# bdina9/qat-vit

Hardware: AMD Instinct MI355X
Metric: images/sec QAT student step (fwd+bwd+allreduce) (higher is better)
Workload: dtype f32 (emulated: int8 MFMA for grid x grid products; forward float operands as fp16 hi+lo pairs; backward gradients as ONE fp16 plane scaled per tensor - 2^-12 per element, <= 4e-4 relative L2 per stage against the fp32 reference, bf16-pair fallback on overflow; fp32 / exact-integer accumulate)

## Files before the change

qat-vit_amd/csrc/f16strip.hip:

```cpp
#include <stdlib.h>

#include "qv_common.h"
#include "qv_kernels.h"

namespace qv {

typedef int i32x4 __attribute__((ext_vector_type(4)));
typedef float f32x4 __attribute__((ext_vector_type(4)));
typedef _Float16 f16x8 __attribute__((ext_vector_type(8)));
typedef __attribute__((address_space(3))) void lds_void;

struct F16StripArgs {
    const _Float16* A;
    const i32x4* Bf;
    int M, N, lda;
    const float* s1;
    const float* s2;
    const float* qp;
    int qmin, qmax;
    const float* colscale;
    const uint8_t* code8;
    const uint8_t* mask;
    int ldc;
    _Float16* out;
    const float* o16_mul;
    uint32_t* o16_amax;
};

typedef int v4i32 __attribute__((ext_vector_type(4)));
__device__ inline v4i32 fs_rsrc(const void* base, int64_t bytes) {
    const uint64_t b = reinterpret_cast<uint64_t>(base);
    const uint32_t n = bytes > 0xffffffffll ? 0xffffffffu : (uint32_t)bytes;
    return (v4i32){(int)(uint32_t)b, (int)(uint32_t)(b >> 32), (int)n, 0x00020000};
}
__device__ inline void fs_dma16(v4i32 rsrc, const char* lds_dst, uint32_t voff) {
    const uint32_t m = __builtin_amdgcn_readfirstlane((uint32_t)reinterpret_cast<uintptr_t>((lds_void*)lds_dst));
    uint32_t keep;
    asm volatile("s_mov_b32 %0, m0\n\ts_mov_b32 m0, %2\n\ts_nop 0\n\tbuffer_load_dwordx4 %1, %3, 0 offen lds\n\ts_mov_b32 m0, %0"
                 : "=&s"(keep)
                 : "v"(voff), "s"(m), "s"(rsrc)
                 : "memory");
}

__device__ inline int fstrip_off(int row, int chunk) {
    const int R = row >> 1;
    return R * 128 + (((((row & 1) << 2) | chunk) ^ (R & 7)) << 4);
}

template <int NTL>
__global__ __launch_bounds__(768, 3) void k_f16_strip_gelu_bwd(const F16StripArgs p) {
    constexpr int NWV = 12, TM = 7, TNT = 2, WC = 32, BMV = 104, KT = 12, PF = 3, NT_ = NWV * 64, BN = 384;
    constexpr int IMGA = 16 * TM * 64, LA = KT * IMGA;
    constexpr int NC = NTL * BN;
    constexpr int WCODE = 16 * TM * WC;
    constexpr int CH = 1, OROW = 80, WOUT = 16 * CH * OROW;
    extern __shared__ __attribute__((aligned(16))) char smem[];
    char* sA = smem;
    float* sCs = reinterpret_cast<float*>(smem + LA);
    float* sLut = sCs + NC;
    char* sCodeAll = reinterpret_cast<char*>(sLut + 256);
    char* sOutAll = sCodeAll + NWV * WCODE;
    const int tid = threadIdx.x, lane = tid & 63;
    const int wave = __builtin_amdgcn_readfirstlane(tid >> 6);
    const int r = lane & 15, g = lane >> 4;
    const int m0 = blockIdx.x * BMV;

    {
        const int64_t abytes = (int64_t)p.M * p.lda * 2;
        const __amdgpu_buffer_rsrc_t rA = __builtin_amdgcn_make_buffer_rsrc(const_cast<_Float16*>(p.A), 0, abytes > 0xffffffffll ? 0xffffffffu : (uint32_t)abytes, 0x00020000);
        const int lR = lane >> 3, lL = (lane & 7) ^ lR;
        const int prow = 2 * lR + (lL >> 2), pk = lL & 3;
#pragma unroll
        for (int kt = 0; kt < KT; ++kt) {
            const int q = wave;
            if (q < TM) {
                const uint32_t off = (uint32_t)(((int64_t)(m0 + q * 16 + prow) * p.lda) * 2 + kt * 64 + pk * 16);
                __builtin_amdgcn_raw_ptr_buffer_load_lds(rA, (lds_void*)(sA + kt * IMGA + q * 1024), 16, off, 0, 0, 0);
            }
        }
    }
    const __amdgpu_buffer_rsrc_t rB = __builtin_amdgcn_make_buffer_rsrc(const_cast<i32x4*>(p.Bf), 0, (uint32_t)((int64_t)p.N * (KT * 64)), 0x00020000);
    const int f0 = wave * TNT;
    auto load_b = [&](int nt, int kt, i32x4 (&b)[TNT]) {
#pragma unroll
        for (int j = 0; j < TNT; ++j) {
            const int f = f0 + nt * 24 + j;
            const auto v = __builtin_amdgcn_raw_buffer_load_b128(rB, lane * 16, (((f / 3) * KT + kt) * 3 + f % 3) * 1024, 0);
            b[j] = __builtin_bit_cast(i32x4, v);
        }
    };
    i32x4 bb[2][TNT];
    load_b(0, 0, bb[0]);
    const v4i32 rC = fs_rsrc(p.code8, (int64_t)p.M * p.ldc);
    char* const sCode = sCodeAll + wave * WCODE;
    auto load_codes = [&](int nt) {
#pragma unroll
        for (int pc = 0; pc < 4; ++pc) {
            const int row = pc * 32 + (lane >> 1);
            if (pc < 3 || lane < 32) {
                const uint32_t off = (uint32_t)((int64_t)(m0 + row) * p.ldc + nt * BN + wave * WC + (lane & 1) * 16);
                fs_dma16(rC, sCode + pc * 1024, off);
            }
        }
    };
    load_codes(0);
    for (int c = tid; c < NC; c += NT_) sCs[c] = p.colscale ? p.colscale[c] : 1.0f;
    if (tid <= p.qmax - p.qmin) sLut[tid] = gelu_bwd(((float)(tid + p.qmin) - p.qp[2]) * p.qp[0]);
    const float alpha = (p.s1 ? *p.s1 : 1.0f) * (p.s2 ? *p.s2 : 1.0f);
    const float mul = *p.o16_mul;
    float am = 0.f;
    asm volatile("s_waitcnt vmcnt(0) lgkmcnt(0)" ::: "memory");
    __builtin_amdgcn_s_barrier();
    asm volatile("" ::: "memory");

    f32x4 acc[TM][TNT];
#pragma clang loop unroll(disable)
    for (int nt = 0; nt < NTL; ++nt) {
        auto kstep = [&](int kt, const i32x4 (&bc)[TNT]) {
            __builtin_amdgcn_sched_barrier(0);
            int opaque = 0;
            asm volatile("" : "+v"(opaque));
            const char* st = sA + opaque + kt * IMGA + fstrip_off(r, g);
            i32x4 af[PF];
#pragma unroll
            for (int i = 0; i < PF - 1; ++i) af[i] = *reinterpret_cast<const i32x4*>(st + 1024 * i);
#pragma unroll
            for (int i = 0; i < TM; ++i) {
                __builtin_amdgcn_sched_barrier(0);
                if (i + PF - 1 < TM) af[(i + PF - 1) % PF] = *reinterpret_cast<const i32x4*>(st + 1024 * (i + PF - 1));
#pragma unroll
                for (int j = 0; j < TNT; ++j)
                    acc[i][j] = __builtin_amdgcn_mfma_f32_16x16x32_f16(__builtin_bit_cast(f16x8, bc[j]), __builtin_bit_cast(f16x8, af[i % PF]),
                                                                       kt == 0 ? f32x4{0.f, 0.f, 0.f, 0.f} : acc[i][j], 0, 0, 0);
            }
        };
        __builtin_amdgcn_s_setprio(2);
#pragma unroll
        for (int kt = 0; kt < KT; ++kt) {
            if (kt + 1 < KT) load_b(nt, kt + 1, bb[(kt + 1) & 1]);
            else if (nt + 1 < NTL) load_b(nt + 1, 0, bb[0]);
            kstep(kt, bb[kt & 1]);
        }
        __builtin_amdgcn_sched_barrier(0);
        if (((wave >> 2) + nt) % 3 == 0) __builtin_amdgcn_s_setprio(1); else __builtin_amdgcn_s_setprio(0);

        int tid2 = threadIdx.x;
        asm volatile("" : "+v"(tid2));
        const int lane2 = tid2 & 63, r2 = lane2 & 15, g2 = lane2 >> 4;
        char* const sOut = sOutAll + wave * WOUT;
        const int colbase = nt * BN + wave * WC;
        uint32_t mword[TM];
#pragma unroll
        for (int i = 0; i < TM; ++i) {
            const int row = m0 + 16 * i + r2;
            mword[i] = row < p.M ? *reinterpret_cast<const uint32_t*>(p.mask + ((int64_t)row * p.ldc + colbase) / 8) : 0u;
        }
        asm volatile("s_waitcnt vmcnt(0)" ::: "memory");
#pragma unroll
        for (int c0 = 0; c0 < TM; c0 += CH) {
            const int nf = TM - c0 < CH ? TM - c0 : CH;
#pragma unroll
            for (int ii = 0; ii < CH; ++ii) {
                if (ii >= nf) continue;
                const int i = c0 + ii, rl = 16 * ii + r2;
#pragma unroll
                for (int j = 0; j < TNT; ++j) {
                    const uint32_t cd = *reinterpret_cast<const uint32_t*>(sCode + (16 * i + r2) * WC + 16 * j + 4 * g2);
                    const float4 cs = *reinterpret_cast<const float4*>(sCs + colbase + 16 * j + 4 * g2);
                    const float sv[4] = {cs.x, cs.y, cs.z, cs.w};
                    const uint32_t mb = mword[i] >> (16 * j + 4 * g2);
                    float o[4];
#pragma unroll
                    for (int e = 0; e < 4; ++e) {
                        const float v = acc[i][j][e] * alpha + 0.0f;
                        const float dg = sLut[(cd >> (8 * e)) & 0xffu];
                        o[e] = ((mb >> e) & 1u) ? v * dg * sv[e] : 0.f;
                    }
                    am = fmaxf(fmaxf(am, fmaxf(fabsf(o[0]), fabsf(o[1]))), fmaxf(fabsf(o[2]), fabsf(o[3])));
                    *reinterpret_cast<uint2*>(sOut + rl * OROW + (16 * j + 4 * g2) * 2) = make_uint2(pk_f16(o[0] * mul, o[1] * mul), pk_f16(o[2] * mul, o[3] * mul));
                }
            }
            asm volatile("s_waitcnt lgkmcnt(0)" ::: "memory");
            {
                const int rl = lane2 >> 2, c = lane2 & 3;
                const int lrow = 16 * c0 + rl, row = m0 + lrow;
                const uint4 v = *reinterpret_cast<const uint4*>(sOut + rl * OROW + 16 * c);
                if (lrow < BMV && row < p.M) *reinterpret_cast<uint4*>(p.out + (int64_t)row * p.ldc + colbase + 8 * c) = v;
            }
            asm volatile("" ::: "memory");
        }
        if (nt + 1 < NTL) {
            asm volatile("s_waitcnt lgkmcnt(0)" ::: "memory");
            load_codes(nt + 1);
        }
    }
    am = wave_max(am);
    if (lane == 0) atomicMax(p.o16_amax + (blockIdx.x & (kDyAmaxSlots - 1)) * kDyAmaxStride, __builtin_bit_cast(uint32_t, am));
}

bool launch_f16_strip_gelu_bwd(const void* A16, const void* B16f, float* , int M, int N, int K, int lda, int ldc, const float* s1, const float* s2, hipStream_t st,
                               const NTPost* post) {
    if (!knobs().f16_strip || !A16 || !B16f || !post || post->mode != 9 || K != 384 || N != 4 * 384 || lda % 8 != 0 || ldc % 128 != 0 || !post->qp || !post->out_hi ||
        !post->code8 || !post->code_mask || !post->o16_mul || !post->o16_amax || post->qmax - post->qmin >= 256)
        return false;
    if ((int64_t)M * lda * 2 >= (1ll << 32) || (int64_t)M * ldc >= (1ll << 32)) return false;
    F16StripArgs a{};
    a.A = reinterpret_cast<const _Float16*>(A16); a.Bf = reinterpret_cast<const i32x4*>(B16f); a.M = M; a.N = N; a.lda = lda; a.s1 = s1; a.s2 = s2;
    a.qp = post->qp; a.qmin = post->qmin; a.qmax = post->qmax; a.colscale = post->colscale;
    a.code8 = reinterpret_cast<const uint8_t*>(post->code8); a.mask = reinterpret_cast<const uint8_t*>(post->code_mask); a.ldc = ldc;
    a.out = reinterpret_cast<_Float16*>(post->out_hi); a.o16_mul = post->o16_mul; a.o16_amax = post->o16_amax;
    constexpr int kLds = 12 * 16 * 7 * 64 + 4 * 384 * 4 + 1024 + 12 * (16 * 7 * 32) + 12 * (16 * 80);
    static_assert(kLds <= 160 * 1024, "LDS");
    static bool once = ((void)hipFuncSetAttribute(reinterpret_cast<const void*>(k_f16_strip_gelu_bwd<4>), hipFuncAttributeMaxDynamicSharedMemorySize, kLds), true);
    (void)once;
    k_f16_strip_gelu_bwd<4><<<cdiv(M, 104), 768, kLds, st>>>(a);
    return true;
}

}
```

Baseline: 15800.

## Make f16 strip GELU-bwd kernel persistent with balanced strips and prefetch

Replaces the fixed grid of 104-row strips with a persistent grid capped at the CU count. Each block walks several equal-sized strips, with row count computed from M so the load balances across rounds. The next strip's A tile, first B fragment and codes are loaded during the epilogue of the current strip, and code reads and LUT gathers in the epilogue are software-pipelined. This aims to cut launch tail imbalance and expose prefetch overlap, at the cost of an extra barrier and more complex synchronization around reuse of shared memory.

```diff
diff --git a/qat-vit_amd/csrc/f16strip.hip b/qat-vit_amd/csrc/f16strip.hip
--- a/qat-vit_amd/csrc/f16strip.hip
+++ b/qat-vit_amd/csrc/f16strip.hip
@@ -14,6 +14,7 @@
     const _Float16* A;
     const i32x4* Bf;
     int M, N, lda;
+    int rows, strips;
     const float* s1;
     const float* s2;
     const float* qp;
@@ -49,11 +50,11 @@
 
 template <int NTL>
 __global__ __launch_bounds__(768, 3) void k_f16_strip_gelu_bwd(const F16StripArgs p) {
-    constexpr int NWV = 12, TM = 7, TNT = 2, WC = 32, BMV = 104, KT = 12, PF = 3, NT_ = NWV * 64, BN = 384;
+    constexpr int NWV = 12, TM = 7, TNT = 2, WC = 32, KT = 12, PF = 3, NT_ = NWV * 64, BN = 384;
     constexpr int IMGA = 16 * TM * 64, LA = KT * IMGA;
     constexpr int NC = NTL * BN;
     constexpr int WCODE = 16 * TM * WC;
-    constexpr int CH = 1, OROW = 80, WOUT = 16 * CH * OROW;
+    constexpr int OROW = 80, WOUT = 16 * OROW;
     extern __shared__ __attribute__((aligned(16))) char smem[];
     char* sA = smem;
     float* sCs = reinterpret_cast<float*>(smem + LA);
@@ -63,22 +64,18 @@
     const int tid = threadIdx.x, lane = tid & 63;
     const int wave = __builtin_amdgcn_readfirstlane(tid >> 6);
     const int r = lane & 15, g = lane >> 4;
-    const int m0 = blockIdx.x * BMV;
-
-    {
-        const int64_t abytes = (int64_t)p.M * p.lda * 2;
-        const __amdgpu_buffer_rsrc_t rA = __builtin_amdgcn_make_buffer_rsrc(const_cast<_Float16*>(p.A), 0, abytes > 0xffffffffll ? 0xffffffffu : (uint32_t)abytes, 0x00020000);
+    const int rows = p.rows;
+
+    const v4i32 rA = fs_rsrc(p.A, (int64_t)p.M * p.lda * 2);
+    auto load_strip = [&](int m0) {
         const int lR = lane >> 3, lL = (lane & 7) ^ lR;
         const int prow = 2 * lR + (lL >> 2), pk = lL & 3;
-#pragma unroll
-        for (int kt = 0; kt < KT; ++kt) {
-            const int q = wave;
-            if (q < TM) {
-                const uint32_t off = (uint32_t)(((int64_t)(m0 + q * 16 + prow) * p.lda) * 2 + kt * 64 + pk * 16);
-                __builtin_amdgcn_raw_ptr_buffer_load_lds(rA, (lds_void*)(sA + kt * IMGA + q * 1024), 16, off, 0, 0, 0);
-            }
-        }
-    }
+        if (wave < TM) {
+            const uint32_t base = (uint32_t)(((int64_t)(m0 + wave * 16 + prow) * p.lda) * 2 + pk * 16);
+#pragma unroll
+            for (int kt = 0; kt < KT; ++kt) fs_dma16(rA, sA + kt * IMGA + wave * 1024, base + kt * 64);
+        }
+    };
     const __amdgpu_buffer_rsrc_t rB = __builtin_amdgcn_make_buffer_rsrc(const_cast<i32x4*>(p.Bf), 0, (uint32_t)((int64_t)p.N * (KT * 64)), 0x00020000);
     const int f0 = wave * TNT;
     auto load_b = [&](int nt, int kt, i32x4 (&b)[TNT]) {
@@ -89,11 +86,9 @@
             b[j] = __builtin_bit_cast(i32x4, v);
         }
     };
-    i32x4 bb[2][TNT];
-    load_b(0, 0, bb[0]);
     const v4i32 rC = fs_rsrc(p.code8, (int64_t)p.M * p.ldc);
     char* const sCode = sCodeAll + wave * WCODE;
-    auto load_codes = [&](int nt) {
+    auto load_codes = [&](int m0, int nt) {
 #pragma unroll
         for (int pc = 0; pc < 4; ++pc) {
             const int row = pc * 32 + (lane >> 1);
@@ -103,96 +98,135 @@
             }
         }
     };
-    load_codes(0);
+    int s = blockIdx.x, m0 = s * rows;
+    load_strip(m0);
+    i32x4 bb[2][TNT];
+    load_b(0, 0, bb[0]);
+    load_codes(m0, 0);
     for (int c = tid; c < NC; c += NT_) sCs[c] = p.colscale ? p.colscale[c] : 1.0f;
     if (tid <= p.qmax - p.qmin) sLut[tid] = gelu_bwd(((float)(tid + p.qmin) - p.qp[2]) * p.qp[0]);
     const float alpha = (p.s1 ? *p.s1 : 1.0f) * (p.s2 ? *p.s2 : 1.0f);
     const float mul = *p.o16_mul;
     float am = 0.f;
-    asm volatile("s_waitcnt vmcnt(0) lgkmcnt(0)" ::: "memory");
-    __builtin_amdgcn_s_barrier();
-    asm volatile("" ::: "memory");
-
-    f32x4 acc[TM][TNT];
+
 #pragma clang loop unroll(disable)
-    for (int nt = 0; nt < NTL; ++nt) {
-        auto kstep = [&](int kt, const i32x4 (&bc)[TNT]) {
+    for (;;) {
+        asm volatile("s_waitcnt vmcnt(0) lgkmcnt(0)" ::: "memory");
+        __builtin_amdgcn_s_barrier();
+        asm volatile("" ::: "memory");
+        const int sn = s + (int)gridDim.x;
+        const bool more = sn < p.strips && sn * rows < p.M;
+        const int m1 = sn * rows;
+
+        f32x4 acc[TM][TNT];
+#pragma clang loop unroll(disable)
+        for (int nt = 0; nt < NTL; ++nt) {
+            auto kstep = [&](int kt, const i32x4 (&bc)[TNT]) {
+                __builtin_amdgcn_sched_barrier(0);
+                int opaque = 0;
+                asm volatile("" : "+v"(opaque));
+                const char* st = sA + opaque + kt * IMGA + fstrip_off(r, g);
+                i32x4 af[PF];
+#pragma unroll
+                for (int i = 0; i < PF - 1; ++i) af[i] = *reinterpret_cast<const i32x4*>(st + 1024 * i);
+#pragma unroll
+                for (int i = 0; i < TM; ++i) {
+                    __builtin_amdgcn_sched_barrier(0);
+                    if (i + PF - 1 < TM) af[(i + PF - 1) % PF] = *reinterpret_cast<const i32x4*>(st + 1024 * (i + PF - 1));
+#pragma unroll
+                    for (int j = 0; j < TNT; ++j)
+                        acc[i][j] = __builtin_amdgcn_mfma_f32_16x16x32_f16(__builtin_bit_cast(f16x8, bc[j]), __builtin_bit_cast(f16x8, af[i % PF]),
+                                                                           kt == 0 ? f32x4{0.f, 0.f, 0.f, 0.f} : acc[i][j], 0, 0, 0);
+                }
+            };
+            __builtin_amdgcn_s_setprio(2);
+#pragma unroll
+            for (int kt = 0; kt < KT; ++kt) {
+                if (kt + 1 < KT) load_b(nt, kt + 1, bb[(kt + 1) & 1]);
+                else if (nt + 1 < NTL || more) load_b(nt + 1 < NTL ? nt + 1 : 0, 0, bb[0]);
+                kstep(kt, bb[kt & 1]);
+            }
             __builtin_amdgcn_sched_barrier(0);
-            int opaque = 0;
-            asm volatile("" : "+v"(opaque));
-            const char* st = sA + opaque + kt * IMGA + fstrip_off(r, g);
-            i32x4 af[PF];
-#pragma unroll
-            for (int i = 0; i < PF - 1; ++i) af[i] = *reinterpret_cast<const i32x4*>(st + 1024 * i);
+            if (((wave >> 2) + nt) % 3 == 0) __builtin_amdgcn_s_setprio(1); else __builtin_amdgcn_s_setprio(0);
+
+            int tid2 = threadIdx.x;
+            asm volatile("" : "+v"(tid2));
+            const int lane2 = tid2 & 63, r2 = lane2 & 15, g2 = lane2 >> 4;
+            char* const sOut = sOutAll + wave * WOUT;
+            const int colbase = nt * BN + wave * WC;
+            uint32_t mword[TM];
 #pragma unroll
             for (int i = 0; i < TM; ++i) {
-                __builtin_amdgcn_sched_barrier(0);
-                if (i + PF - 1 < TM) af[(i + PF - 1) % PF] = *reinterpret_cast<const i32x4*>(st + 1024 * (i + PF - 1));
+                const int row = m0 + 16 * i + r2;
+                mword[i] = row < p.M ? *reinterpret_cast<const uint32_t*>(p.mask + ((int64_t)row * p.ldc + colbase) / 8) : 0u;
+            }
+            asm volatile("s_waitcnt vmcnt(0)" ::: "memory");
+#pragma unroll
+            for (int i = 0; i < TM; ++i) asm volatile("" : "+v"(mword[i]));
+            if (nt + 1 == NTL && more) {
+                __builtin_amdgcn_s_barrier();
+                asm volatile("" ::: "memory");
+                load_strip(m1);
+            }
+            float sv[TNT][4];
+#pragma unroll
+            for (int j = 0; j < TNT; ++j) {
+                const float4 cs = *reinterpret_cast<const float4*>(sCs + colbase + 16 * j + 4 * g2);
+                sv[j][0] = cs.x; sv[j][1] = cs.y; sv[j][2] = cs.z; sv[j][3] = cs.w;
+            }
+            uint32_t cd[TNT];
+            float dg[TNT][4];
+            auto read_codes = [&](int i) {
+#pragma unroll
+                for (int j = 0; j < TNT; ++j) cd[j] = *reinterpret_cast<const uint32_t*>(sCode + (16 * i + r2) * WC + 16 * j + 4 * g2);
+            };
+            auto gather = [&]() {
 #pragma unroll
                 for (int j = 0; j < TNT; ++j)
-                    acc[i][j] = __builtin_amdgcn_mfma_f32_16x16x32_f16(__builtin_bit_cast(f16x8, bc[j]), __builtin_bit_cast(f16x8, af[i % PF]),
-                                                                       kt == 0 ? f32x4{0.f, 0.f, 0.f, 0.f} : acc[i][j], 0, 0, 0);
-            }
-        };
-        __builtin_amdgcn_s_setprio(2);
-#pragma unroll
-        for (int kt = 0; kt < KT; ++kt) {
-            if (kt + 1 < KT) load_b(nt, kt + 1, bb[(kt + 1) & 1]);
-            else if (nt + 1 < NTL) load_b(nt + 1, 0, bb[0]);
-            kstep(kt, bb[kt & 1]);
-        }
-        __builtin_amdgcn_sched_barrier(0);
-        if (((wave >> 2) + nt) % 3 == 0) __builtin_amdgcn_s_setprio(1); else __builtin_amdgcn_s_setprio(0);
-
-        int tid2 = threadIdx.x;
-        asm volatile("" : "+v"(tid2));
-        const int lane2 = tid2 & 63, r2 = lane2 & 15, g2 = lane2 >> 4;
-        char* const sOut = sOutAll + wave * WOUT;
-        const int colbase = nt * BN + wave * WC;
-        uint32_t mword[TM];
-#pragma unroll
-        for (int i = 0; i < TM; ++i) {
-            const int row = m0 + 16 * i + r2;
-            mword[i] = row < p.M ? *reinterpret_cast<const uint32_t*>(p.mask + ((int64_t)row * p.ldc + colbase) / 8) : 0u;
-        }
-        asm volatile("s_waitcnt vmcnt(0)" ::: "memory");
-#pragma unroll
-        for (int c0 = 0; c0 < TM; c0 += CH) {
-            const int nf = TM - c0 < CH ? TM - c0 : CH;
-#pragma unroll
-            for (int ii = 0; ii < CH; ++ii) {
-                if (ii >= nf) continue;
-                const int i = c0 + ii, rl = 16 * ii + r2;
+#pragma unroll
+                    for (int e = 0; e < 4; ++e) dg[j][e] = sLut[(cd[j] >> (8 * e)) & 0xffu];
+            };
+            read_codes(0);
+            gather();
+#pragma unroll
+            for (int i = 0; i < TM; ++i) {
+                if (i + 1 < TM) read_codes(i + 1);
+                asm volatile("" : "+v"(dg[0][0]), "+v"(dg[0][1]), "+v"(dg[0][2]), "+v"(dg[0][3]), "+v"(dg[1][0]), "+v"(dg[1][1]), "+v"(dg[1][2]), "+v"(dg[1][3]));
+                float dgi[TNT][4];
+#pragma unroll
+                for (int j = 0; j < TNT; ++j)
+#pragma unroll
+                    for (int e = 0; e < 4; ++e) dgi[j][e] = dg[j][e];
 #pragma unroll
                 for (int j = 0; j < TNT; ++j) {
-                    const uint32_t cd = *reinterpret_cast<const uint32_t*>(sCode + (16 * i + r2) * WC + 16 * j + 4 * g2);
-                    const float4 cs = *reinterpret_cast<const float4*>(sCs + colbase + 16 * j + 4 * g2);
-                    const float sv[4] = {cs.x, cs.y, cs.z, cs.w};
                     const uint32_t mb = mword[i] >> (16 * j + 4 * g2);
                     float o[4];
 #pragma unroll
                     for (int e = 0; e < 4; ++e) {
                         const float v = acc[i][j][e] * alpha + 0.0f;
-                        const float dg = sLut[(cd >> (8 * e)) & 0xffu];
-                        o[e] = ((mb >> e) & 1u) ? v * dg * sv[e] : 0.f;
+                        const float t = v * dgi[j][e] * sv[j][e];
+                        o[e] = ((mb >> e) & 1u) ? t : 0.f;
                     }
                     am = fmaxf(fmaxf(am, fmaxf(fabsf(o[0]), fabsf(o[1]))), fmaxf(fabsf(o[2]), fabsf(o[3])));
-                    *reinterpret_cast<uint2*>(sOut + rl * OROW + (16 * j + 4 * g2) * 2) = make_uint2(pk_f16(o[0] * mul, o[1] * mul), pk_f16(o[2] * mul, o[3] * mul));
+                    *reinterpret_cast<uint2*>(sOut + r2 * OROW + (16 * j + 4 * g2) * 2) = make_uint2(pk_f16(o[0] * mul, o[1] * mul), pk_f16(o[2] * mul, o[3] * mul));
                 }
-            }
-            asm volatile("s_waitcnt lgkmcnt(0)" ::: "memory");
-            {
-                const int rl = lane2 >> 2, c = lane2 & 3;
-                const int lrow = 16 * c0 + rl, row = m0 + lrow;
-                const uint4 v = *reinterpret_cast<const uint4*>(sOut + rl * OROW + 16 * c);
-                if (lrow < BMV && row < p.M) *reinterpret_cast<uint4*>(p.out + (int64_t)row * p.ldc + colbase + 8 * c) = v;
-            }
-            asm volatile("" ::: "memory");
-        }
-        if (nt + 1 < NTL) {
-            asm volatile("s_waitcnt lgkmcnt(0)" ::: "memory");
-            load_codes(nt + 1);
-        }
+                asm volatile("s_waitcnt lgkmcnt(0)" ::: "memory");
+                if (i + 1 < TM) gather();
+                {
+                    const int rl = lane2 >> 2, c = lane2 & 3;
+                    const int lrow = 16 * i + rl, row = m0 + lrow;
+                    const uint4 v = *reinterpret_cast<const uint4*>(sOut + rl * OROW + 16 * c);
+                    if (lrow < rows && row < p.M) *reinterpret_cast<uint4*>(p.out + (int64_t)row * p.ldc + colbase + 8 * c) = v;
+                }
+                asm volatile("" ::: "memory");
+            }
+            if (nt + 1 < NTL || more) {
+                asm volatile("s_waitcnt lgkmcnt(0)" ::: "memory");
+                if (nt + 1 < NTL) load_codes(m0, nt + 1); else load_codes(m1, 0);
+            }
+        }
+        if (!more) break;
+        s = sn; m0 = m1;
     }
     am = wave_max(am);
     if (lane == 0) atomicMax(p.o16_amax + (blockIdx.x & (kDyAmaxSlots - 1)) * kDyAmaxStride, __builtin_bit_cast(uint32_t, am));
@@ -201,11 +235,18 @@
 bool launch_f16_strip_gelu_bwd(const void* A16, const void* B16f, float* , int M, int N, int K, int lda, int ldc, const float* s1, const float* s2, hipStream_t st,
                                const NTPost* post) {
     if (!knobs().f16_strip || !A16 || !B16f || !post || post->mode != 9 || K != 384 || N != 4 * 384 || lda % 8 != 0 || ldc % 128 != 0 || !post->qp || !post->out_hi ||
-        !post->code8 || !post->code_mask || !post->o16_mul || !post->o16_amax || post->qmax - post->qmin >= 256)
+        !post->code8 || !post->code_mask || !post->o16_mul || !post->o16_amax || post->qmax - post->qmin >= 256 || M < 1)
         return false;
-    if ((int64_t)M * lda * 2 >= (1ll << 32) || (int64_t)M * ldc >= (1ll << 32)) return false;
+    if ((int64_t)(M + 112) * lda * 2 >= (1ll << 32) || (int64_t)(M + 112) * ldc >= (1ll << 32)) return false;
+    static int cus = 0;
+    if (!cus) {
+        int dev = 0;
+        if (hipGetDevice(&dev) != hipSuccess || hipDeviceGetAttribute(&cus, hipDeviceAttributeMultiprocessorCount, dev) != hipSuccess || cus < 1 || cus > 256) cus = 256;
+    }
+    const int need = cdiv(M, 112), grid = need < cus ? need : cus, rounds = cdiv(need, grid);
     F16StripArgs a{};
     a.A = reinterpret_cast<const _Float16*>(A16); a.Bf = reinterpret_cast<const i32x4*>(B16f); a.M = M; a.N = N; a.lda = lda; a.s1 = s1; a.s2 = s2;
+    a.strips = grid * rounds; a.rows = cdiv(M, a.strips);
     a.qp = post->qp; a.qmin = post->qmin; a.qmax = post->qmax; a.colscale = post->colscale;
     a.code8 = reinterpret_cast<const uint8_t*>(post->code8); a.mask = reinterpret_cast<const uint8_t*>(post->code_mask); a.ldc = ldc;
     a.out = reinterpret_cast<_Float16*>(post->out_hi); a.o16_mul = post->o16_mul; a.o16_amax = post->o16_amax;
@@ -213,7 +254,7 @@
     static_assert(kLds <= 160 * 1024, "LDS");
     static bool once = ((void)hipFuncSetAttribute(reinterpret_cast<const void*>(k_f16_strip_gelu_bwd<4>), hipFuncAttributeMaxDynamicSharedMemorySize, kLds), true);
     (void)once;
-    k_f16_strip_gelu_bwd<4><<<cdiv(M, 104), 768, kLds, st>>>(a);
+    k_f16_strip_gelu_bwd<4><<<grid, 768, kLds, st>>>(a);
     return true;
 }
 
```

New measurement: 15890, median of 6. About the same (+0.6%).
